# vwxyzjn/cleanrl

Hardware: NVIDIA H100
Metric: env steps/sec (SPS) PPO Breakout num_envs=1024 (higher is better)
Workload: dtype bf16

## Files before the change

cleanrl_b200/csrc/tc_common.cuh:

```cuda
#pragma once
#include <cuda_bf16.h>
#include <cstdint>
#include "tc_wgmma.cuh"

namespace b200rl { namespace tc {

__device__ __forceinline__ uint32_t smem_u32(const void* p) {
    return static_cast<uint32_t>(__cvta_generic_to_shared(p));
}

__device__ __forceinline__ void mbar_init(uint64_t* bar, uint32_t count) {
    asm volatile("mbarrier.init.shared::cta.b64 [%0], %1;" ::"r"(smem_u32(bar)), "r"(count) : "memory");
}
__device__ __forceinline__ void fence_barrier_init() {
    asm volatile("fence.mbarrier_init.release.cluster;" ::: "memory");
}
__device__ __forceinline__ bool mbar_try_wait(uint64_t* bar, uint32_t parity) {
    uint32_t ok;
    asm volatile(
        "{\n\t.reg .pred p;\n\t"
        "mbarrier.try_wait.parity.shared::cta.b64 p, [%1], %2;\n\t"
        "selp.u32 %0, 1, 0, p;\n\t}\n"
        : "=r"(ok)
        : "r"(smem_u32(bar)), "r"(parity)
        : "memory");
    return ok != 0;
}
#ifndef B200RL_WAIT_MODE
#define B200RL_WAIT_MODE 0
#endif
__device__ __forceinline__ bool mbar_try_wait_hint(uint64_t* bar, uint32_t parity, uint32_t ns) {
    uint32_t ok;
    asm volatile(
        "{\n\t.reg .pred p;\n\t"
        "mbarrier.try_wait.parity.shared::cta.b64 p, [%1], %2, %3;\n\t"
        "selp.u32 %0, 1, 0, p;\n\t}\n"
        : "=r"(ok)
        : "r"(smem_u32(bar)), "r"(parity), "r"(ns)
        : "memory");
    return ok != 0;
}
__device__ __forceinline__ void mbar_wait(uint64_t* bar, uint32_t parity) {
    if (mbar_try_wait(bar, parity)) return;
    const long long t0 = clock64();
#if B200RL_WAIT_MODE == 1
    while (!mbar_try_wait_hint(bar, parity, 1000000u)) {
#elif B200RL_WAIT_MODE == 2
    while (!mbar_try_wait(bar, parity)) {
        __nanosleep(40);
#else
    while (!mbar_try_wait(bar, parity)) {
#endif
        if (clock64() - t0 > (1ll << 33)) __trap();
    }
}

__device__ __forceinline__ void mbar_wait2(uint64_t* bar_a, uint32_t parity_a, uint64_t* bar_b, uint32_t parity_b) {
    const bool a = mbar_try_wait(bar_a, parity_a), b = mbar_try_wait(bar_b, parity_b);
    if (a && b) return;
    if (!a) mbar_wait(bar_a, parity_a);
    if (!b) mbar_wait(bar_b, parity_b);
}

__device__ __forceinline__ void st_global_32b(void* p, const int4& a, const int4& b) {
    reinterpret_cast<int4*>(p)[0] = a;
    reinterpret_cast<int4*>(p)[1] = b;
}

__device__ __forceinline__ void fence_proxy_async_smem() {
    asm volatile("fence.proxy.async.shared::cta;" ::: "memory");
}

constexpr uint64_t kDescSwizzle128 = 1ull << 62;
constexpr uint64_t kDescSwizzle64 = 2ull << 62;

__device__ __forceinline__ uint64_t desc_kmajor(uint32_t smem_addr) {
    return (uint64_t)((smem_addr & 0x3FFFFu) >> 4) | (1ull << 16) | (64ull << 32) | kDescSwizzle128;
}
__device__ __forceinline__ uint64_t desc_mnmajor(uint32_t smem_addr, uint32_t lbo_bytes) {
    return (uint64_t)((smem_addr & 0x3FFFFu) >> 4) | ((uint64_t)((lbo_bytes >> 4) & 0x3FFF) << 16) | (64ull << 32) |
           kDescSwizzle128;
}

template <int R>
__device__ __forceinline__ void stage_acc(float* st, int ld, int wg_tid, const float (&d)[R]) {
    const int row = ((wg_tid >> 5) << 4) + ((wg_tid & 31) >> 2), col = (wg_tid & 3) * 2;
#pragma unroll
    for (int j = 0; j < R / 4; ++j) {
        *reinterpret_cast<float2*>(st + row * ld + 8 * j + col) = make_float2(d[4 * j], d[4 * j + 1]);
        *reinterpret_cast<float2*>(st + (row + 8) * ld + 8 * j + col) = make_float2(d[4 * j + 2], d[4 * j + 3]);
    }
}
__device__ __forceinline__ void named_bar(int id, int n) { asm volatile("bar.sync %0, %1;" ::"r"(id), "r"(n) : "memory"); }

__device__ __forceinline__ uint32_t img_off(int r, int c) { return (uint32_t)(r * 128 + ((c ^ (r & 7)) << 4)); }

__device__ __forceinline__ uint32_t pack_bf16x2_relu(float lo, float hi) {
    uint32_t d;
    asm("cvt.rn.relu.bf16x2.f32 %0, %1, %2;" : "=r"(d) : "f"(hi), "f"(lo));
    return d;
}
__device__ __forceinline__ uint32_t pack_bf16x2(float lo, float hi) {
    __nv_bfloat162 v = __floats2bfloat162_rn(lo, hi);
    return *reinterpret_cast<uint32_t*>(&v);
}

}}

namespace b200rl { namespace tc {
__device__ __forceinline__ void cp_async16(uint32_t smem_addr, const void* gptr, uint32_t src_bytes) {
    asm volatile("cp.async.cg.shared.global [%0], [%1], 16, %2;" ::"r"(smem_addr), "l"(gptr), "r"(src_bytes) : "memory");
}
__device__ __forceinline__ void cp_async_commit() { asm volatile("cp.async.commit_group;" ::: "memory"); }
template <int N>
__device__ __forceinline__ void cp_async_wait() { asm volatile("cp.async.wait_group %0;" ::"n"(N) : "memory"); }
__device__ __forceinline__ void mbar_arrive(uint64_t* bar) {
    asm volatile("mbarrier.arrive.shared::cta.b64 _, [%0];" ::"r"(smem_u32(bar)) : "memory");
}
template <int R> __device__ __forceinline__ void setmaxnreg_dec() { asm volatile("setmaxnreg.dec.sync.aligned.u32 %0;" ::"n"(R)); }
template <int R> __device__ __forceinline__ void setmaxnreg_inc() { asm volatile("setmaxnreg.inc.sync.aligned.u32 %0;" ::"n"(R)); }
}}

namespace b200rl { namespace tc {
__device__ __forceinline__ void tma_load_2d(uint32_t smem_dst, const void* tmap, int x, int y, uint64_t* bar) {
    asm volatile("cp.async.bulk.tensor.2d.shared::cluster.global.mbarrier::complete_tx::bytes [%0], [%1, {%2, %3}], [%4];"
                 ::"r"(smem_dst), "l"(reinterpret_cast<uint64_t>(tmap)), "r"(x), "r"(y), "r"(smem_u32(bar))
                 : "memory");
}
__device__ __forceinline__ void tma_load_3d(uint32_t smem_dst, const void* tmap, int x, int y, int z, uint64_t* bar) {
    asm volatile("cp.async.bulk.tensor.3d.shared::cluster.global.mbarrier::complete_tx::bytes [%0], [%1, {%2, %3, %4}], [%5];"
                 ::"r"(smem_dst), "l"(reinterpret_cast<uint64_t>(tmap)), "r"(x), "r"(y), "r"(z), "r"(smem_u32(bar))
                 : "memory");
}
__device__ __forceinline__ void mbar_arrive_expect_tx(uint64_t* bar, uint32_t bytes) {
    asm volatile("mbarrier.arrive.expect_tx.shared::cta.b64 _, [%0], %1;" ::"r"(smem_u32(bar)), "r"(bytes) : "memory");
}
__device__ __forceinline__ void tma_prefetch_desc(const void* tmap) {
    asm volatile("prefetch.tensormap [%0];" ::"l"(reinterpret_cast<uint64_t>(tmap)) : "memory");
}
}}
```

cleanrl_b200/csrc/tc_gemm_tma.cuh:

```cuda
#pragma once
#include "tc_base.cuh"

namespace b200rl {
using namespace tc;

struct KGemmParams {
    const void* A;
    int64_t M;
    int nchunks;
    const bf16* Bw;
    int N;
    bf16* out;
    int ldo;
    const float* bias;
    float scale;
    int relu;
    const uint32_t* mask_bits;
    uint32_t* mask_out;
    int dual_dact3;
    bf16* out2;
    float* out_f32;
    int ncols_f32;
};

constexpr int kGemmThreads = 384;
constexpr int kGemmRegsProducer = 40, kGemmRegsMma = 232;
static_assert(128 * kGemmRegsProducer + 256 * kGemmRegsMma <= 65536, "register budgets exceed the SM");
template <int BN>
__host__ __device__ constexpr size_t gemm_acc_bytes() { return (size_t)8 * 8 * (BN + 4) * sizeof(float); }

template <int BN, int STAGES>
__device__ __forceinline__ void gemm_tile_mma(float (&d)[BN / 64][BN / 2], uint32_t ring, uint64_t* full_bar,
                                              uint64_t* empty_bar, uint32_t q0, int nch, int tid) {
    constexpr int MH = BN / 64;
    constexpr int A_BYTES = BN * 128;
    constexpr int STAGE_BYTES = A_BYTES + BN * 128;
    auto chunk = [&](int j) {
        const uint32_t q = q0 + (uint32_t)j, s = q % STAGES;
        mbar_wait(&full_bar[s], (q / STAGES) & 1);
        wgmma_fence();
        const uint32_t stage_addr = ring + s * STAGE_BYTES;
        const uint64_t b = desc_kmajor(stage_addr + A_BYTES);
#pragma unroll
        for (int h = 0; h < MH; ++h) {
            const uint64_t a = desc_kmajor(stage_addr + h * 64 * 128);
#pragma unroll
            for (int kk = 0; kk < 4; ++kk) WgmmaBf16<BN, 0, 0>::mma(d[h], a + 2 * kk, b + 2 * kk, (j | kk) != 0 ? 1u : 0u);
        }
        wgmma_commit();
    };
    for (int j = 0; j + 1 < nch; ++j) {
        chunk(j);
        wgmma_wait<1>();
        if (j > 0 && (tid & 31) == 0) mbar_arrive(&empty_bar[(q0 + (uint32_t)j - 1u) % STAGES]);
    }
    chunk(nch - 1);
    wgmma_wait<0>();
#pragma unroll
    for (int h = 0; h < MH; ++h) wgmma_fence_operands(d[h]);
    if ((tid & 31) == 0) {
        if (nch > 1) mbar_arrive(&empty_bar[(q0 + (uint32_t)nch - 2u) % STAGES]);
        mbar_arrive(&empty_bar[(q0 + (uint32_t)nch - 1u) % STAGES]);
    }
}

template <int BN, int STAGES>
__global__ void __launch_bounds__(kGemmThreads, 1) tc_gemm_tma(const __grid_constant__ CUtensorMap tmA,
                                                               const __grid_constant__ CUtensorMap tmB,
                                                               const KGemmParams p, int total_tiles, int ntiles_n) {
    static_assert(BN == 64 || BN == 128, "one epilogue lane per row and 32-column group of 8 rows");
    constexpr int MH = BN / 64;
    constexpr int A_BYTES = BN * 128;
    constexpr int STAGE_BYTES = A_BYTES + BN * 128;
    constexpr int LDA = BN + 4;
    constexpr int NW = BN / 32;
    constexpr int PR = BN / 8;
    extern __shared__ uint8_t smem_raw[];
    __shared__ uint64_t full_bar[2][STAGES], empty_bar[2][STAGES];
    uint8_t* smem = reinterpret_cast<uint8_t*>((reinterpret_cast<uintptr_t>(smem_raw) + 1023) & ~uintptr_t(1023));
    float* sAcc = reinterpret_cast<float*>(smem + (size_t)2 * STAGES * STAGE_BYTES);
    const int tid = threadIdx.x, warp = tid >> 5, lane = tid & 31;
    const int nch = p.nchunks;
    if (tid == 0) {
        for (int w = 0; w < 2; ++w)
            for (int s = 0; s < STAGES; ++s) { mbar_init(&full_bar[w][s], 1); mbar_init(&empty_bar[w][s], 4); }
        fence_barrier_init();
        tma_prefetch_desc(&tmA);
        tma_prefetch_desc(&tmB);
    }
    __syncthreads();

    if (warp < 4) {
        setmaxnreg_dec<kGemmRegsProducer>();
        if (warp < 2 && lane == 0) {
            const int w = warp;
            uint8_t* ring = smem + (size_t)w * STAGES * STAGE_BYTES;
            uint32_t q = 0;
            for (int tile = blockIdx.x + w * gridDim.x; tile < total_tiles; tile += 2 * gridDim.x) {
                const int mt = tile / ntiles_n, n0 = (tile - mt * ntiles_n) * BN;
                for (int j = 0; j < nch; ++j, ++q) {
                    const uint32_t s = q % STAGES;
                    if (q >= (uint32_t)STAGES) mbar_wait(&empty_bar[w][s], ((q / STAGES) - 1) & 1);
                    const uint32_t dst = smem_u32(ring + (size_t)s * STAGE_BYTES);
                    mbar_arrive_expect_tx(&full_bar[w][s], STAGE_BYTES);
                    tma_load_2d(dst, &tmA, j * 64, mt * BN, &full_bar[w][s]);
                    tma_load_2d(dst + A_BYTES, &tmB, j * 64, n0, &full_bar[w][s]);
                }
            }
        }
    } else {
        setmaxnreg_inc<kGemmRegsMma>();
        const int wg = (warp - 4) >> 2, ww = (warp - 4) & 3;
        float* st = sAcc + (warp - 4) * 8 * LDA;
        const uint32_t ring = smem_u32(smem + (size_t)wg * STAGES * STAGE_BYTES);
        const int nwords = p.N >> 5;
        const int er = lane & 7, eg = lane >> 3;
        uint32_t q = 0;
        for (int tile = blockIdx.x + wg * gridDim.x; tile < total_tiles; tile += 2 * gridDim.x, q += (uint32_t)nch) {
            const int mt = tile / ntiles_n, n0 = (tile - mt * ntiles_n) * BN;
            float d[MH][BN / 2];
#pragma unroll
            for (int h = 0; h < MH; ++h)
#pragma unroll
                for (int e = 0; e < BN / 2; ++e) d[h][e] = 0.f;
            gemm_tile_mma<BN, STAGES>(d, ring, full_bar[wg], empty_bar[wg], q, nch, tid);
#pragma unroll
            for (int pass = 0; pass < 2 * MH; ++pass) {
                const int h = pass >> 1, hi = pass & 1;
                const int row0 = mt * BN + 64 * h + 16 * ww + 8 * hi;
#pragma unroll
                for (int j = 0; j < BN / 8; ++j)
                    *reinterpret_cast<float2*>(st + (lane >> 2) * LDA + 8 * j + 2 * (lane & 3)) =
                        make_float2(d[h][4 * j + 2 * hi], d[h][4 * j + 2 * hi + 1]);
                __syncwarp();
                const int r = row0 + er, col = n0 + eg * 32;
                const bool live = eg < NW && r < (int)p.M && col < p.N;
                int4 w[4];
                if (live) {
                    const int64_t wb = (int64_t)r * nwords + (col >> 5);
                    uint32_t v[32];
#pragma unroll
                    for (int e = 0; e < 8; ++e) {
                        const float4 f = *reinterpret_cast<const float4*>(st + er * LDA + eg * 32 + 4 * e);
                        v[4 * e] = __float_as_uint(f.x); v[4 * e + 1] = __float_as_uint(f.y);
                        v[4 * e + 2] = __float_as_uint(f.z); v[4 * e + 3] = __float_as_uint(f.w);
                    }
                    const uint32_t mbw = p.mask_bits != nullptr ? __ldg(p.mask_bits + wb) : 0xFFFFFFFFu;
                    if (p.bias) {
                        const float4* bp = reinterpret_cast<const float4*>(p.bias + col);
#pragma unroll
                        for (int e = 0; e < 8; ++e) {
                            const float4 bv = __ldg(bp + e);
                            v[4 * e] = __float_as_uint(fmaf(__uint_as_float(v[4 * e]), p.scale, bv.x));
                            v[4 * e + 1] = __float_as_uint(fmaf(__uint_as_float(v[4 * e + 1]), p.scale, bv.y));
                            v[4 * e + 2] = __float_as_uint(fmaf(__uint_as_float(v[4 * e + 2]), p.scale, bv.z));
                            v[4 * e + 3] = __float_as_uint(fmaf(__uint_as_float(v[4 * e + 3]), p.scale, bv.w));
                        }
                    } else {
#pragma unroll
                        for (int e = 0; e < 32; ++e) v[e] = __float_as_uint(__uint_as_float(v[e]) * p.scale);
                    }
                    if (p.relu) {
                        uint32_t bits = 0u;
#pragma unroll
                        for (int e = 0; e < 32; ++e) {
                            const bool pos = __uint_as_float(v[e]) > 0.f;
                            bits |= (pos ? 1u : 0u) << e;
                            v[e] = pos ? v[e] : 0u;
                        }
                        if (p.mask_out) p.mask_out[wb] = bits;
                    }
                    if (p.mask_bits) {
#pragma unroll
                        for (int e = 0; e < 32; ++e) if (!((mbw >> e) & 1u)) v[e] = 0u;
                    }
                    if (p.out_f32) {
                        float* dst = p.out_f32 + (int64_t)r * p.ldo + col;
#pragma unroll
                        for (int e = 0; e < 32; ++e) if (col + e < p.ncols_f32) dst[e] = __uint_as_float(v[e]);
                    }
#pragma unroll
                    for (int e = 0; e < 4; ++e) {
                        w[e].x = (int)pack_bf16x2(__uint_as_float(v[8 * e]), __uint_as_float(v[8 * e + 1]));
                        w[e].y = (int)pack_bf16x2(__uint_as_float(v[8 * e + 2]), __uint_as_float(v[8 * e + 3]));
                        w[e].z = (int)pack_bf16x2(__uint_as_float(v[8 * e + 4]), __uint_as_float(v[8 * e + 5]));
                        w[e].w = (int)pack_bf16x2(__uint_as_float(v[8 * e + 6]), __uint_as_float(v[8 * e + 7]));
                    }
                }
                __syncwarp();
                if (live) {
                    int4* brow = reinterpret_cast<int4*>(st + er * LDA) + 4 * eg;
#pragma unroll
                    for (int e = 0; e < 4; ++e) brow[e] = w[e];
                }
                __syncwarp();
                if (p.out_f32 == nullptr) {
#pragma unroll
                    for (int k = lane; k < 8 * PR; k += 32) {
                        const int rr = k / PR, pc = k % PR;
                        const int rs = row0 + rr, cs = n0 + pc * 8;
                        if (rs >= (int)p.M || cs >= p.N) continue;
                        const int4 val = reinterpret_cast<const int4*>(st + rr * LDA)[pc];
                        if (p.dual_dact3) {
                            const int px = cs >> 6;
                            const int oy = px / 7, ox = px - oy * 7;
                            *reinterpret_cast<int4*>(p.out + ((int64_t)rs * 81 + oy * 9 + ox) * 64 + (cs & 63)) = val;
                            *reinterpret_cast<int4*>(p.out2 + ((int64_t)rs * 121 + (oy + 2) * 11 + ox + 2) * 64 + (cs & 63)) = val;
                        } else {
                            *reinterpret_cast<int4*>(p.out + (int64_t)rs * p.ldo + cs) = val;
                        }
                    }
                }
                __syncwarp();
            }
        }
    }
}

template <int BN, int STAGES>
static int launch_gemm_tma(const KGemmParams& p, cudaStream_t s, const char* what) {
    const size_t smem = (size_t)2 * STAGES * (BN * 128 + BN * 128) + gemm_acc_bytes<BN>() + 1024;
    static SmemAttrCache attr;
    int rc;
    if (p.N % 64 != 0 || BN % 64 != 0) return fail(B200RL_ERR_INVALID_ARGUMENT, "%s: N must be a multiple of 64", what);
    if (p.nchunks < 1) return fail(B200RL_ERR_INVALID_ARGUMENT, "%s: K must be at least 64", what);
    if (p.out_f32 == nullptr && !p.dual_dact3 && p.ldo % 8 != 0)
        return fail(B200RL_ERR_INVALID_ARGUMENT, "%s: output pitch must be a multiple of 8 (16-byte stores)", what);
    if ((rc = attr.ensure(tc_gemm_tma<BN, STAGES>, smem, what))) return rc;
    CUtensorMap tmA, tmB;
    const int64_t K = (int64_t)p.nchunks * 64;
    if ((rc = make_tmap_2d(&tmA, p.A, p.M, K, BN, what))) return rc;
    if ((rc = make_tmap_2d(&tmB, p.Bw, p.N, K, BN, what))) return rc;
    const int ntn = (int)ceil_div(p.N, BN);
    const int total = (int)ceil_div(p.M, BN) * ntn;
    int grid = num_sms();
    if (grid > total) grid = total;
    tc_gemm_tma<BN, STAGES><<<grid, kGemmThreads, smem, s>>>(tmA, tmB, p, total, ntn);
    return check_launch(what);
}

constexpr int kWgradTmaThreads = 384;
constexpr int kFcWgradXChunks = 2, kFcWgradYChunks = 4;
static __global__ void __launch_bounds__(kWgradTmaThreads, 1) tc_wgrad_tma(const __grid_constant__ CUtensorMap tmX,
                                                                    const __grid_constant__ CUtensorMap tmY,
                                                                    int64_t M, int64_t rows_per_cta, float* ws) {
    constexpr int R = 64, STAGES = 4, nxc = kFcWgradXChunks, nyc = kFcWgradYChunks, NY = 64 * nyc;
    extern __shared__ uint8_t smem_raw[];
    __shared__ uint64_t full_bar[STAGES], empty_bar[STAGES];
    uint8_t* smem = reinterpret_cast<uint8_t*>((reinterpret_cast<uintptr_t>(smem_raw) + 1023) & ~uintptr_t(1023));
    const int tid = threadIdx.x, warp = tid >> 5;
    const int xc0 = blockIdx.y * nxc, yc0 = blockIdx.z * nyc;
    constexpr int chunk_img = R * 128;
    constexpr int stage_bytes = (nxc + nyc) * chunk_img;
    if (tid == 0) {
        for (int s = 0; s < STAGES; ++s) { mbar_init(&full_bar[s], 1); mbar_init(&empty_bar[s], 8); }
        fence_barrier_init();
        tma_prefetch_desc(&tmX);
        tma_prefetch_desc(&tmY);
    }
    __syncthreads();
    const int64_t m_begin = (int64_t)blockIdx.x * rows_per_cta;
    int64_t m_end = m_begin + rows_per_cta;
    if (m_end > M) m_end = M;
    const int nsteps = m_end > m_begin ? (int)((m_end - m_begin + R - 1) / R) : 0;

    if (warp == 0 && (tid & 31) == 0) {
        for (int it = 0; it < nsteps; ++it) {
            const int s = it % STAGES;
            if (it >= STAGES) mbar_wait(&empty_bar[s], ((it / STAGES) - 1) & 1);
            const uint32_t dst = smem_u32(smem + (size_t)s * stage_bytes);
            const int m0 = (int)(m_begin + (int64_t)it * R);
            mbar_arrive_expect_tx(&full_bar[s], (uint32_t)stage_bytes);
            for (int c = 0; c < nxc; ++c) tma_load_2d(dst + c * chunk_img, &tmX, (xc0 + c) * 64, m0, &full_bar[s]);
            for (int c = 0; c < nyc; ++c) tma_load_2d(dst + (nxc + c) * chunk_img, &tmY, (yc0 + c) * 64, m0, &full_bar[s]);
        }
    } else if (warp >= 4) {
        const int wg = (warp - 4) >> 2, wt = tid & 127;
        float d[NY / 2];
#pragma unroll
        for (int e = 0; e < NY / 2; ++e) d[e] = 0.f;
        auto step = [&](int it) {
            const int s = it % STAGES;
            mbar_wait(&full_bar[s], (it / STAGES) & 1);
            wgmma_fence();
            const uint32_t xa = smem_u32(smem + (size_t)s * stage_bytes), ya = xa + nxc * chunk_img;
#pragma unroll
            for (int kk = 0; kk < R / 16; ++kk) {
                const uint64_t adesc = desc_mnmajor(xa + wg * chunk_img + kk * 2048, chunk_img);
                const uint64_t bdesc = desc_mnmajor(ya + kk * 2048, chunk_img);
                WgmmaBf16<NY, 1, 1>::mma(d, adesc, bdesc, (it | kk) != 0 ? 1u : 0u);
            }
            wgmma_commit();
        };
        for (int it = 0; it + 1 < nsteps; ++it) {
            step(it);
            wgmma_wait<1>();
            if (it > 0 && (tid & 31) == 0) mbar_arrive(&empty_bar[(it - 1) % STAGES]);
        }
        step(nsteps - 1);
        wgmma_wait<0>();
        wgmma_fence_operands(d);
        const int64_t NYtot = (int64_t)gridDim.z * nyc * 64;
        const int64_t KXtot = (int64_t)gridDim.y * nxc * 64;
        float* wsb = ws + (int64_t)blockIdx.x * KXtot * NYtot;
        const int row = ((wt >> 5) << 4) + ((wt & 31) >> 2), col = (wt & 3) * 2;
        float* d0 = wsb + ((int64_t)xc0 * 64 + wg * 64 + row) * NYtot + (int64_t)yc0 * 64 + col;
        float* d8 = d0 + 8 * NYtot;
#pragma unroll
        for (int j = 0; j < NY / 8; ++j) {
            *reinterpret_cast<float2*>(d0 + 8 * j) = make_float2(d[4 * j], d[4 * j + 1]);
            *reinterpret_cast<float2*>(d8 + 8 * j) = make_float2(d[4 * j + 2], d[4 * j + 3]);
        }
    }
}

static int64_t round_up(int64_t a, int64_t b) { return ceil_div(a, b) * b; }
struct WPlan { int64_t rows_per_cta; int splits; };
static WPlan wgrad_plan(int64_t M, int target_ctas, int quantum = 32) {
    WPlan w;
    w.rows_per_cta = round_up(ceil_div(M, target_ctas), quantum);
    if (w.rows_per_cta < quantum) w.rows_per_cta = quantum;
    w.splits = (int)ceil_div(M, w.rows_per_cta);
    if (w.splits < 1) w.splits = 1;
    return w;
}
constexpr int kFcSplits = 8;

static size_t wgrad_tma_bytes(int64_t M, int xcols, int ycols) {
    return (size_t)wgrad_plan(M, kFcSplits, 64).splits * xcols * round_up(ycols, 64 * kFcWgradYChunks) * sizeof(float);
}
static int launch_wgrad_tma(const void* X, int xcols, const void* Y, int ycols, int64_t M, float* ws, cudaStream_t s,
                            const char* what) {
    if (xcols % (64 * kFcWgradXChunks) != 0) return fail(B200RL_ERR_INVALID_ARGUMENT, "%s: X columns must be a multiple of 128", what);
    const WPlan pl = wgrad_plan(M, kFcSplits, 64);
    if (M < 1) {
        const cudaError_t e = cudaMemsetAsync(ws, 0, wgrad_tma_bytes(M, xcols, ycols), s);
        if (e != cudaSuccess) return fail(B200RL_ERR_CUDA, "%s: cudaMemsetAsync: %s", what, cudaGetErrorString(e));
        return pl.splits;
    }
    CUtensorMap tmX, tmY;
    int rc;
    if ((rc = make_tmap_2d(&tmX, X, M, xcols, 64, what))) return rc;
    if ((rc = make_tmap_2d(&tmY, Y, M, ycols, 64, what))) return rc;
    const size_t smem = (size_t)4 * (kFcWgradXChunks + kFcWgradYChunks) * 64 * 128 + 1024;
    static SmemAttrCache attr;
    if ((rc = attr.ensure(tc_wgrad_tma, smem, what))) return rc;
    const dim3 grid(pl.splits, xcols / (64 * kFcWgradXChunks), (unsigned)ceil_div(ycols, 64 * kFcWgradYChunks));
    tc_wgrad_tma<<<grid, kWgradTmaThreads, smem, s>>>(tmX, tmY, M, pl.rows_per_cta, ws);
    if ((rc = check_launch(what))) return rc;
    return pl.splits;
}

}
```

Baseline: 1.427 million.

## Share one TMA ring between ping-pong consumer warpgroups with named-barrier handoff

Replaces the two per-warpgroup TMA producer rings with a single producer and a shared ring of twice the stages. The two consumer warpgroups alternate tiles and pass a named barrier to each other so they issue MMAs in turn, while the other warpgroup runs its epilogue. The mask-bit loads for the epilogue are also hoisted ahead of the MMA loop to hide their latency. The ordering adds serialization between warpgroups, and a single producer thread could limit load issue rate.

```diff
diff --git a/cleanrl_b200/csrc/tc_common.cuh b/cleanrl_b200/csrc/tc_common.cuh
--- a/cleanrl_b200/csrc/tc_common.cuh
+++ b/cleanrl_b200/csrc/tc_common.cuh
@@ -92,6 +92,7 @@
     }
 }
 __device__ __forceinline__ void named_bar(int id, int n) { asm volatile("bar.sync %0, %1;" ::"r"(id), "r"(n) : "memory"); }
+__device__ __forceinline__ void named_bar_arrive(int id, int n) { asm volatile("bar.arrive %0, %1;" ::"r"(id), "r"(n) : "memory"); }
 
 __device__ __forceinline__ uint32_t img_off(int r, int c) { return (uint32_t)(r * 128 + ((c ^ (r & 7)) << 4)); }
 
diff --git a/cleanrl_b200/csrc/tc_gemm_tma.cuh b/cleanrl_b200/csrc/tc_gemm_tma.cuh
--- a/cleanrl_b200/csrc/tc_gemm_tma.cuh
+++ b/cleanrl_b200/csrc/tc_gemm_tma.cuh
@@ -75,15 +75,15 @@
     constexpr int LDA = BN + 4;
     constexpr int NW = BN / 32;
     constexpr int PR = BN / 8;
+    constexpr int NS = 2 * STAGES;
     extern __shared__ uint8_t smem_raw[];
-    __shared__ uint64_t full_bar[2][STAGES], empty_bar[2][STAGES];
+    __shared__ uint64_t full_bar[NS], empty_bar[NS];
     uint8_t* smem = reinterpret_cast<uint8_t*>((reinterpret_cast<uintptr_t>(smem_raw) + 1023) & ~uintptr_t(1023));
-    float* sAcc = reinterpret_cast<float*>(smem + (size_t)2 * STAGES * STAGE_BYTES);
+    float* sAcc = reinterpret_cast<float*>(smem + (size_t)NS * STAGE_BYTES);
     const int tid = threadIdx.x, warp = tid >> 5, lane = tid & 31;
     const int nch = p.nchunks;
     if (tid == 0) {
-        for (int w = 0; w < 2; ++w)
-            for (int s = 0; s < STAGES; ++s) { mbar_init(&full_bar[w][s], 1); mbar_init(&empty_bar[w][s], 4); }
+        for (int s = 0; s < NS; ++s) { mbar_init(&full_bar[s], 1); mbar_init(&empty_bar[s], 4); }
         fence_barrier_init();
         tma_prefetch_desc(&tmA);
         tma_prefetch_desc(&tmB);
@@ -92,19 +92,17 @@
 
     if (warp < 4) {
         setmaxnreg_dec<kGemmRegsProducer>();
-        if (warp < 2 && lane == 0) {
-            const int w = warp;
-            uint8_t* ring = smem + (size_t)w * STAGES * STAGE_BYTES;
+        if (warp == 0 && lane == 0) {
             uint32_t q = 0;
-            for (int tile = blockIdx.x + w * gridDim.x; tile < total_tiles; tile += 2 * gridDim.x) {
+            for (int tile = blockIdx.x; tile < total_tiles; tile += gridDim.x) {
                 const int mt = tile / ntiles_n, n0 = (tile - mt * ntiles_n) * BN;
                 for (int j = 0; j < nch; ++j, ++q) {
-                    const uint32_t s = q % STAGES;
-                    if (q >= (uint32_t)STAGES) mbar_wait(&empty_bar[w][s], ((q / STAGES) - 1) & 1);
-                    const uint32_t dst = smem_u32(ring + (size_t)s * STAGE_BYTES);
-                    mbar_arrive_expect_tx(&full_bar[w][s], STAGE_BYTES);
-                    tma_load_2d(dst, &tmA, j * 64, mt * BN, &full_bar[w][s]);
-                    tma_load_2d(dst + A_BYTES, &tmB, j * 64, n0, &full_bar[w][s]);
+                    const uint32_t s = q % NS;
+                    if (q >= (uint32_t)NS) mbar_wait(&empty_bar[s], ((q / NS) - 1) & 1);
+                    const uint32_t dst = smem_u32(smem + (size_t)s * STAGE_BYTES);
+                    mbar_arrive_expect_tx(&full_bar[s], STAGE_BYTES);
+                    tma_load_2d(dst, &tmA, j * 64, mt * BN, &full_bar[s]);
+                    tma_load_2d(dst + A_BYTES, &tmB, j * 64, n0, &full_bar[s]);
                 }
             }
         }
@@ -112,18 +110,27 @@
         setmaxnreg_inc<kGemmRegsMma>();
         const int wg = (warp - 4) >> 2, ww = (warp - 4) & 3;
         float* st = sAcc + (warp - 4) * 8 * LDA;
-        const uint32_t ring = smem_u32(smem + (size_t)wg * STAGES * STAGE_BYTES);
+        const uint32_t ring = smem_u32(smem);
         const int nwords = p.N >> 5;
         const int er = lane & 7, eg = lane >> 3;
-        uint32_t q = 0;
-        for (int tile = blockIdx.x + wg * gridDim.x; tile < total_tiles; tile += 2 * gridDim.x, q += (uint32_t)nch) {
+        uint32_t q = (uint32_t)(wg * nch);
+        for (int tile = blockIdx.x + wg * gridDim.x; tile < total_tiles; tile += 2 * gridDim.x, q += (uint32_t)(2 * nch)) {
             const int mt = tile / ntiles_n, n0 = (tile - mt * ntiles_n) * BN;
+            uint32_t mbw[2 * MH];
+#pragma unroll
+            for (int pass = 0; pass < 2 * MH; ++pass) {
+                const int r = mt * BN + 64 * (pass >> 1) + 16 * ww + 8 * (pass & 1) + er, col = n0 + eg * 32;
+                mbw[pass] = p.mask_bits != nullptr && eg < NW && r < (int)p.M && col < p.N
+                                ? __ldg(p.mask_bits + (int64_t)r * nwords + (col >> 5)) : 0xFFFFFFFFu;
+            }
             float d[MH][BN / 2];
 #pragma unroll
             for (int h = 0; h < MH; ++h)
 #pragma unroll
                 for (int e = 0; e < BN / 2; ++e) d[h][e] = 0.f;
-            gemm_tile_mma<BN, STAGES>(d, ring, full_bar[wg], empty_bar[wg], q, nch, tid);
+            if (tile != (int)blockIdx.x) named_bar(1 + wg, 256);
+            gemm_tile_mma<BN, NS>(d, ring, full_bar, empty_bar, q, nch, tid);
+            if (tile + (int)gridDim.x < total_tiles) named_bar_arrive(2 - wg, 256);
 #pragma unroll
             for (int pass = 0; pass < 2 * MH; ++pass) {
                 const int h = pass >> 1, hi = pass & 1;
@@ -145,7 +152,6 @@
                         v[4 * e] = __float_as_uint(f.x); v[4 * e + 1] = __float_as_uint(f.y);
                         v[4 * e + 2] = __float_as_uint(f.z); v[4 * e + 3] = __float_as_uint(f.w);
                     }
-                    const uint32_t mbw = p.mask_bits != nullptr ? __ldg(p.mask_bits + wb) : 0xFFFFFFFFu;
                     if (p.bias) {
                         const float4* bp = reinterpret_cast<const float4*>(p.bias + col);
 #pragma unroll
@@ -172,7 +178,7 @@
                     }
                     if (p.mask_bits) {
 #pragma unroll
-                        for (int e = 0; e < 32; ++e) if (!((mbw >> e) & 1u)) v[e] = 0u;
+                        for (int e = 0; e < 32; ++e) if (!((mbw[pass] >> e) & 1u)) v[e] = 0u;
                     }
                     if (p.out_f32) {
                         float* dst = p.out_f32 + (int64_t)r * p.ldo + col;
```

Result: faster. 1.442 million, median of 6 (+1.1%).
